# nv-tlabs/InfiniCube

Measured on AMD Instinct MI355X. Metric: denoise steps/sec, 93-frame 480p Wan2.1 buffer-conditioned DiT loop, higher is better.
Workload: dtype bf16

## Files before the change

infinicube_amd/csrc/attention.hip:

```cpp
#include "icv_common.h"


int icv_attn1_dispatch(const void* q, int64_t ldq, const void* k, int64_t ldk, const void* v, int64_t ldv, void* o,
                       int64_t ldo, int64_t Sq, int64_t Skv, int64_t heads, float scale, void* stream);
int icv_attn2_dispatch(const void* q, int64_t ldq, const void* k, int64_t ldk, const void* v, int64_t ldv,
                       void* o, int64_t ldo, float* acc, int64_t ldacc, float* ml, int state_in,
                       int state_out, int64_t Sq, int64_t Skv, int64_t heads, float scale, int var,
                       hipStream_t st);

int icv_attn3_dispatch(const void* q, int64_t ldq, const void* k, int64_t ldk, const void* v, int64_t ldv,
                       void* o, int64_t ldo, float* acc, int64_t ldacc, float* ml, int state_in,
                       int state_out, int64_t Sq, int64_t Skv, int64_t heads, float scale, int var,
                       hipStream_t st);

int icv_attn9_dispatch(const void* q, int64_t ldq, const void* k, int64_t ldk, const void* v, int64_t ldv,
                       void* o, int64_t ldo, float* acc, int64_t ldacc, float* ml, int state_in,
                       int state_out, int64_t Sq, int64_t Skv, int64_t heads, float scale, int var,
                       hipStream_t st);
int icv_attn7p_single(const void* q, int64_t ldq, const void* k, int64_t ldk, const void* v, int64_t ldv, void* o, int64_t ldo, float* acc,
                      int64_t ldacc, float* ml, int state_in, int state_out, int64_t Sq, int64_t Skv, int64_t heads, float scale, hipStream_t st);
int icv_attn7q_single(const void* q, int64_t ldq, const void* k, int64_t ldk, const void* v, int64_t ldv, void* o, int64_t ldo, float* acc,
                      int64_t ldacc, float* ml, int state_in, int state_out, int64_t Sq, int64_t Skv, int64_t heads, float scale, int variant,
                      hipStream_t st);
int icv_attn7_dispatch(const void* q, int64_t ldq, const void* k, int64_t ldk, const void* v, int64_t ldv,
// ... 70 lines not shown
                                 int64_t Skv, int64_t heads, float scale, void* stream) {
  ICV_REQUIRE(q && k && v && o, "icv_attention_fwd: null pointer");
  ICV_REQUIRE(Sq > 0 && Skv > 0 && heads > 0, "icv_attention_fwd: empty problem (Sq=%lld Skv=%lld heads=%lld)", (long long)Sq, (long long)Skv, (long long)heads);
  ICV_REQUIRE(ldq % 8 == 0 && ldk % 8 == 0 && ldv % 8 == 0 && ldo % 4 == 0, "icv_attention_fwd: leading dims must keep 16-byte row alignment");
  if (icv_get_option_int("attn_kernel", ATTN_KERNEL_DEFAULT) != 1)
    return attn_route(q, ldq, k, ldk, v, ldv, o, ldo, nullptr, 0, nullptr, 0, 0, Sq, Skv, heads, scale, (hipStream_t)stream);
#ifdef ICV_EXPERIMENTS
  return icv_attn1_dispatch(q, ldq, k, ldk, v, ldv, o, ldo, Sq, Skv, heads, scale, stream);
#else
  icv_set_error("attn_kernel 1 is an experiment: rebuild libicvideo with ICV_EXPERIMENTS=1");
  return 1;
#endif
}

extern "C" int icv_attention_fwd_add(const void* q, int64_t ldq, const void* k, int64_t ldk,
                                     const void* v, int64_t ldv, void* o, int64_t ldo, int64_t Sq,
                                     int64_t Skv, int64_t heads, float scale, void* stream) {
  ICV_REQUIRE(q && k && v && o, "icv_attention_fwd_add: null pointer");
  ICV_REQUIRE(Sq > 0 && Skv > 0 && heads > 0, "icv_attention_fwd_add: empty problem (Sq=%lld Skv=%lld heads=%lld)", (long long)Sq, (long long)Skv, (long long)heads);
  ICV_REQUIRE(ldq % 8 == 0 && ldk % 8 == 0 && ldv % 8 == 0 && ldo % 4 == 0, "icv_attention_fwd_add: leading dims must keep 16-byte row alignment");
  return attn_route(q, ldq, k, ldk, v, ldv, o, ldo, nullptr, 0, nullptr, 0, 2, Sq, Skv, heads, scale, (hipStream_t)stream);
}

namespace {
unsigned long long* g_trace = nullptr;
int g_trace_cap = 0;
}
unsigned long long* icv_attention_trace_buffer(int* capacity) {
  *capacity = g_trace_cap;
  return g_trace;
}
extern "C" int icv_attention_trace(void* buf, int64_t capacity) {
  ICV_REQUIRE(capacity >= 0 && capacity < (1LL << 31), "icv_attention_trace: bad capacity");
  g_trace = (unsigned long long*)buf;
  g_trace_cap = buf ? (int)capacity : 0;
  return 0;
}
```

infinicube_amd/csrc/attn7.hip:

```cpp
#include "attn_common.h"

namespace att7 {

using attc::D;
using attc::NEG_BIG;
using attc::Params;
using attc::lds_read_tr16;
constexpr int KVB = 64;
constexpr int TILE_BYTES = KVB * D * 2;
constexpr int STAGE_BYTES = 2 * TILE_BYTES;

__device__ __forceinline__ void dma16(const void* gsrc, unsigned lds_dst) {
  unsigned keep;
  asm volatile(
      "s_mov_b32 %0, m0\n\t"
      "s_mov_b32 m0, %2\n\t"
      "s_nop 0\n\t"
      "global_load_lds_dwordx4 %1, off\n\t"
      "s_mov_b32 m0, %0"
      : "=&s"(keep)
      : "v"(gsrc), "s"(lds_dst)
      : "memory");
}

__device__ __forceinline__ void dma16s(const void* base, unsigned off, unsigned lds_dst) {
  unsigned keep;
  asm volatile(
      "s_mov_b32 %0, m0\n\t"
      "s_mov_b32 m0, %3\n\t"
      "s_nop 0\n\t"
      "global_load_lds_dwordx4 %1, %2\n\t"
      "s_mov_b32 m0, %0"
      : "=&s"(keep)
      : "v"(off), "s"(base), "s"(lds_dst)
      : "memory");
}

#ifndef ATTN7_SHORT_DEFAULT
#define ATTN7_SHORT_DEFAULT 1024
#endif

template <int VAR, int NW, int NST>
__global__ __launch_bounds__(NW * 64) __attribute__((amdgpu_waves_per_eu(2))) void attn7_kernel(Params p) {
  constexpr bool STAGGER = VAR & 1, KPREFETCH = VAR & 2, SETPRIO = VAR & 4, DEEP = VAR & 8, UNIT = VAR & 16;
  constexpr bool DSMAJOR = !(VAR & 32);
  constexpr bool PAIR = (VAR & 128) != 0;
  static_assert(!(PAIR && (STAGGER || DEEP)), "the paired schedule has its own DMA distance");
  static_assert(!(STAGGER && DEEP), "the staggered group already runs its DMA three tiles ahead");
  static_assert(NST == 4 || !(PAIR || STAGGER || DEEP), "the two-stage ring has one schedule");
  static_assert(NW == 8 || !STAGGER, "the stagger pairs waves 0-3 with 4-7");
  constexpr int NI = 16 / NW;
  constexpr int QB = NW * 32;
  const float p_lim = __builtin_amdgcn_exp2f(p.thr);
  extern __shared__ __attribute__((aligned(16))) char smem[];
  const int tid = threadIdx.x;
  const int lane = tid & 63;
  const int wave = __builtin_amdgcn_readfirstlane(tid >> 6);
  const int hi = lane >> 5;
  const int l31 = lane & 31;

  int head, qb;
  attc::work_item(p, head, qb);
  const int64_t q0 = (int64_t)qb * QB + wave * 32;
  const unsigned long long t_start = p.trace ? __builtin_amdgcn_s_memrealtime() : 0ull;

  const bf16_t* qh = p.q + (int64_t)head * D;
  const bf16_t* kh = p.k + (int64_t)head * D;
  const bf16_t* vh = p.v + (int64_t)head * D;

  int64_t qr_c = q0 + l31;
  qr_c = qr_c < p.Sq ? qr_c : p.Sq - 1;

  f32x16 ot[4];
  float m_run, l_run;
  attc::load_state(p, qr_c, head, hi, ot, m_run, l_run);
  float m_base = m_run < -1.0e29f ? 0.f : m_run;
  f32x16 cinit;
  const f32x16 zero16 = {0.f, 0.f, 0.f, 0.f, 0.f, 0.f, 0.f, 0.f, 0.f, 0.f, 0.f, 0.f, 0.f, 0.f, 0.f, 0.f};
#pragma unroll
  for (int r = 0; r < 16; ++r) cinit[r] = UNIT ? -m_base : 0.f;

  bf16x8 qf[8];
#define A7_LOAD_Q()                                                                                   \
  {                                                                                                   \
    const bf16_t* qp = qh + qr_c * p.ldq + hi * 8;                                                    \
    _Pragma("unroll") for (int ds = 0; ds < 8; ++ds) qf[ds] = *reinterpret_cast<const bf16x8*>(qp + ds * 16); \
  }
  if (NST != 2) {
    A7_LOAD_Q();
    __builtin_amdgcn_s_waitcnt(0x0F70);
  }

  const int pc = lane & 15;
  const int nt = (int)((p.Skv + KVB - 1) / KVB);
  const unsigned lds_base = (unsigned)(uintptr_t)((__attribute__((address_space(3))) char*)smem);
  int dkey[NI], kcol[NI], vcol[NI];
  unsigned ko[NI], vo[NI];
#pragma unroll
  for (int j = 0; j < NI; ++j) {
    dkey[j] = (wave * NI + j) * 4 + (lane >> 4);
    kcol[j] = (pc ^ (dkey[j] & 15)) * 8;
    vcol[j] = (pc ^ ((dkey[j] & 3) << 2)) * 8;
    ko[j] = (unsigned)(((int64_t)dkey[j] * p.ldk + kcol[j]) * 2);
    vo[j] = (unsigned)(((int64_t)dkey[j] * p.ldv + vcol[j]) * 2);
  }
#define A7_DMA_TILE(T_)                                                                              \
  {                                                                                                  \
    const int tt_ = (T_) < nt ? (T_) : nt - 1;                                                       \
    const unsigned l0_ = lds_base + (unsigned)(((T_) & (NST - 1)) * STAGE_BYTES + (wave * NI) * 1024); \
    if ((int64_t)(tt_ + 1) * KVB <= p.Skv) {                                                         \
      const bf16_t* kt_ = kh + (int64_t)tt_ * KVB * p.ldk;                                           \
      const bf16_t* vt_ = vh + (int64_t)tt_ * KVB * p.ldv;                                           \
      _Pragma("unroll") for (int j_ = 0; j_ < NI; ++j_) dma16s(kt_, ko[j_], l0_ + j_ * 1024);        \
      _Pragma("unroll") for (int j_ = 0; j_ < NI; ++j_) dma16s(vt_, vo[j_], l0_ + TILE_BYTES + j_ * 1024); \
    } else {                                                                                         \
      _Pragma("unroll") for (int j_ = 0; j_ < NI; ++j_) {                                            \
        int64_t r_ = (int64_t)tt_ * KVB + dkey[j_];                                                  \
        r_ = r_ < p.Skv ? r_ : p.Skv - 1;                                                            \
        dma16(kh + r_ * p.ldk + kcol[j_], l0_ + j_ * 1024);                                          \
        dma16(vh + r_ * p.ldv + vcol[j_], l0_ + TILE_BYTES + j_ * 1024);                             \
      }                                                                                              \
    }                                                                                                \
  }
#define A7_VMCNT4()                                              \
  do {                                                           \
// ... 17 lines not shown
    A7_LOAD_Q();
    asm volatile("s_waitcnt vmcnt(0)" ::: "memory");
  } else if (PAIR) asm volatile("s_waitcnt vmcnt(0)" ::: "memory");
  else A7_VMCNT4();
  A7_BARRIER();
  if (grp == 1) {
    A7_DMA_TILE(2);
    A7_VMCNT4();
    A7_BARRIER();
  }

  const int k_row_off = l31 * 256;
  const int k_sw = l31 & 15;
  const int g = lane >> 4, t16 = lane & 15;
  const int v_key_lo = 4 * hi + (t16 >> 2);
  const int v_byte_lo = (g & 1) * 32 + (t16 & 3) * 8;
  const int v_sw = (t16 >> 2) << 6;
  const int ahead = 2 + grp + (DEEP ? 1 : 0);

  auto tile = [&](const int t) __attribute__((always_inline)) {
    const char* ks = smem + (t & (NST - 1)) * STAGE_BYTES;
    const char* vs = ks + TILE_BYTES;
    const int64_t key0 = (int64_t)t * KVB;

    f32x16 st[2];
    const bool no_ref = UNIT && m_run < -1.0e29f;
    if (KPREFETCH) {
      bf16x8 kf[2][8];
#pragma unroll
      for (int kb = 0; kb < 2; ++kb)
#pragma unroll
        for (int ds = 0; ds < 8; ++ds) {
          const int c = ds * 2 + hi;
          kf[kb][ds] = *reinterpret_cast<const bf16x8*>(ks + kb * 8192 + k_row_off + ((c ^ k_sw) << 4));
        }
      __builtin_amdgcn_sched_barrier(0);
      if (SETPRIO) __builtin_amdgcn_s_setprio(1);
#pragma unroll
      for (int ds = 0; ds < 8; ++ds)
#pragma unroll
        for (int kb = 0; kb < 2; ++kb)
          st[kb] = __builtin_amdgcn_mfma_f32_32x32x16_bf16(kf[kb][ds], qf[ds], ds == 0 ? (UNIT ? cinit : zero16) : st[kb], 0, 0, 0);
      if (SETPRIO) __builtin_amdgcn_s_setprio(0);
    } else if (DSMAJOR) {
#pragma unroll
      for (int ds = 0; ds < 8; ++ds)
// ... 103 lines not shown
    }
  } else if (PAIR) {
    for (int t = 0; t < nt; t += 2) {
      if (!(p.ablate & 1)) {
        A7_DMA_TILE(t + 2);
        A7_DMA_TILE(t + 3);
      }
      tile(t);
      if (t + 1 < nt) tile(t + 1);
      asm volatile("s_waitcnt vmcnt(0)" ::: "memory");
      if (!(p.ablate & 2)) A7_BARRIER();
    }
  } else {
    for (int t = 0; t < nt; ++t) {
      if (!(p.ablate & 1)) A7_DMA_TILE(t + ahead);
      tile(t);
      A7_VMCNT4();
      if (!(p.ablate & 2)) A7_BARRIER();
    }
  }
  asm volatile("s_waitcnt vmcnt(0)" ::: "memory");
  if (grp == 0 && STAGGER) A7_BARRIER();

  attc::store_result(p, q0 + l31, head, hi, ot, m_run, l_run);
  if (p.trace && tid == 0 && (int)blockIdx.x < p.trace_cap) {
    unsigned hwid, xcc;
    asm volatile("s_getreg_b32 %0, hwreg(HW_REG_HW_ID)" : "=s"(hwid));
    asm volatile("s_getreg_b32 %0, hwreg(HW_REG_XCC_ID)" : "=s"(xcc));
    unsigned long long* t = p.trace + (size_t)blockIdx.x * 4;
    t[0] = t_start; t[1] = __builtin_amdgcn_s_memrealtime(); t[2] = hwid; t[3] = xcc;
  }
}

template <int VAR, int NW = 8, int NST = 4>
int launch(const Params& p, hipStream_t st) {
  constexpr int LDS_BYTES = NST * STAGE_BYTES;
  static icv_dev_flags attr_set = {};
  if (int rc = icv_ensure_dynamic_lds((const void*)attn7_kernel<VAR, NW, NST>, LDS_BYTES, &attr_set, "attn7")) return rc;
  const int64_t nwg = (int64_t)p.heads * p.nqb;
  hipLaunchKernelGGL((attn7_kernel<VAR, NW, NST>), dim3((unsigned)nwg), dim3(NW * 64), LDS_BYTES, st, p);
  return icv_check_launch("icv_attention(7)");
}

}

int icv_attn7_dispatch(const void* q, int64_t ldq, const void* k, int64_t ldk, const void* v, int64_t ldv,
                       void* o, int64_t ldo, float* acc, int64_t ldacc, float* ml, int state_in,
                       int state_out, int64_t Sq, int64_t Skv, int64_t heads, float scale, int var,
                       hipStream_t st) {
  att7::Params p;
  int short_max = icv_get_option_int("attn7_short", -1);
  if (short_max < 0) short_max = ATTN7_SHORT_DEFAULT;
  const bool short_kv = Skv <= short_max;
  attc::fill_params(p, q, ldq, k, ldk, v, ldv, o, ldo, acc, ldacc, ml, state_in, state_out, Sq, Skv, heads, scale, short_kv ? 128 : 256);
  if (p.sc == 1.0f && icv_get_option_int("attn_unit_scale", 1)) var |= 16;
  p.ablate = icv_get_option_int("attn7_ablate", 0);
  p.trace = icv_attention_trace_buffer(&p.trace_cap);
  if (short_kv) return (var & 16) ? att7::launch<16, 4, 2>(p, st) : att7::launch<0, 4, 2>(p, st);
  switch (var) {
    case 0: return att7::launch<0>(p, st);
    case 1: return att7::launch<1>(p, st);
    case 4: return att7::launch<4>(p, st);
    case 5: return att7::launch<5>(p, st);
    case 6: return att7::launch<6>(p, st);
    case 7: return att7::launch<7>(p, st);
    case 8: return att7::launch<8>(p, st);
    case 24: return att7::launch<24>(p, st);
    case 32: return att7::launch<32>(p, st);
    case 48: return att7::launch<48>(p, st);
    case 128: return att7::launch<128>(p, st);
    case 144: return att7::launch<144>(p, st);
    case 132: return att7::launch<132>(p, st);
    case 148: return att7::launch<148>(p, st);
    case 16: return att7::launch<16>(p, st);
    case 17: return att7::launch<17>(p, st);
    case 20: return att7::launch<20>(p, st);
    case 21: return att7::launch<21>(p, st);
    case 22: return att7::launch<22>(p, st);
    case 23: return att7::launch<23>(p, st);
  }
  icv_set_error("icv_attention_fwd: unknown attn7 variant %d", var);
  return 1;
}
```

infinicube_amd/csrc/attn7p.hip:

```cpp
#include "attn_common.h"

namespace att7p {

using attc::D;
using attc::NEG_BIG;
using attc::lds_read_tr16;
constexpr int KVB = 64;
constexpr int TILE_BYTES = KVB * D * 2;
constexpr int STAGE_BYTES = 2 * TILE_BYTES;
constexpr int NST = 4, NW = 8, NI = 16 / NW, QB = NW * 32;
constexpr int LDS_BYTES = NST * STAGE_BYTES + 64;
constexpr int MAX_PIECES = ICV_ATTN_MAX_PIECES;

struct Piece {
  const bf16_t* k;
  const bf16_t* v;
  int rows;
  int flag;
  unsigned value;
  int pad;
};

struct Params {
  attc::Params a;
// ... 18 lines not shown
      : "v"(gsrc), "s"(lds_dst)
      : "memory");
}

__device__ __forceinline__ void dma16s(const void* base, unsigned off, unsigned lds_dst) {
  unsigned keep;
  asm volatile(
      "s_mov_b32 %0, m0\n\t"
      "s_mov_b32 m0, %3\n\t"
      "s_nop 0\n\t"
      "global_load_lds_dwordx4 %1, %2\n\t"
      "s_mov_b32 m0, %0"
      : "=&s"(keep)
      : "v"(off), "s"(base), "s"(lds_dst)
      : "memory");
}

__device__ __forceinline__ unsigned load_flag_async(const unsigned* f) {
  unsigned v;
  asm volatile("global_load_dword %0, %1, off sc0 sc1" : "=v"(v) : "v"(f) : "memory");
  return v;
}

template <bool UNIT, bool FW = false>
__global__ __launch_bounds__(NW * 64) __attribute__((amdgpu_waves_per_eu(2))) void attn7p_kernel(Params pp) {
  const attc::Params& p = pp.a;
  const float p_lim = __builtin_amdgcn_exp2f(p.thr);
  extern __shared__ __attribute__((aligned(16))) char smem[];
  volatile unsigned* verdict = reinterpret_cast<volatile unsigned*>(smem + NST * STAGE_BYTES);
  const int tid = threadIdx.x;
  const int lane = tid & 63;
  const int wave = __builtin_amdgcn_readfirstlane(tid >> 6);
  const int hi = lane >> 5;
  const int l31 = lane & 31;

  int head, qb;
  attc::work_item(p, head, qb);
  int64_t q0 = (int64_t)qb * QB + wave * 32;
  int64_t q_end = 0;
  int fw_np = 1, fw_a0 = 0, fw_b0 = 0, fw_a1 = 0, fw_b1 = 0;
  if constexpr (FW) {
    const int T = pp.fw_frames, F = pp.fw_frame_rows, W = pp.fw_window, sink = pp.fw_sink;
    const int bpf = (F + QB - 1) / QB;
    const int f = qb / bpf;
    q0 = (int64_t)f * F + (qb - f * bpf) * QB + wave * 32;
    q_end = (int64_t)(f + 1) * F;
    const int lo = f - W > 0 ? f - W : 0;
    const int hi = f + W + 1 < T ? f + W + 1 : T;
    if (sink == 0) {
      fw_a0 = lo; fw_b0 = hi;
    } else if (lo <= sink) {
      fw_a0 = 0; fw_b0 = hi > sink ? hi : sink;
    } else {
      fw_np = 2;
      fw_a0 = 0; fw_b0 = sink;
      fw_a1 = lo; fw_b1 = hi;
    }
  }
  const unsigned long long t_start = p.trace ? __builtin_amdgcn_s_memrealtime() : 0ull;
  const bf16_t* qh = p.q + (int64_t)head * D;
  int64_t qr_c = q0 + l31;
  if constexpr (FW) qr_c = qr_c < q_end ? qr_c : q_end - 1;
  else qr_c = qr_c < p.Sq ? qr_c : p.Sq - 1;

  f32x16 ot[4];
  float m_run, l_run;
  attc::load_state(p, qr_c, head, hi, ot, m_run, l_run);
  float m_base = m_run < -1.0e29f ? 0.f : m_run;
  f32x16 cinit;
  const f32x16 zero16 = {0.f, 0.f, 0.f, 0.f, 0.f, 0.f, 0.f, 0.f, 0.f, 0.f, 0.f, 0.f, 0.f, 0.f, 0.f, 0.f};
#pragma unroll
  for (int r = 0; r < 16; ++r) cinit[r] = UNIT ? -m_base : 0.f;

  bf16x8 qf[8];
  {
    const bf16_t* qp = qh + qr_c * p.ldq + hi * 8;
#pragma unroll
    for (int ds = 0; ds < 8; ++ds) qf[ds] = *reinterpret_cast<const bf16x8*>(qp + ds * 16);
  }
  __builtin_amdgcn_s_waitcnt(0x0F70);

  const int pc = lane & 15;
  const unsigned lds_base = (unsigned)(uintptr_t)((__attribute__((address_space(3))) char*)smem);
  int dkey[NI], kcol[NI], vcol[NI];
  unsigned ko[NI], vo[NI];
#pragma unroll
  for (int j = 0; j < NI; ++j) {
    dkey[j] = (wave * NI + j) * 4 + (lane >> 4);
    kcol[j] = (pc ^ (dkey[j] & 15)) * 8;
    vcol[j] = (pc ^ ((dkey[j] & 3) << 2)) * 8;
    ko[j] = (unsigned)(((int64_t)dkey[j] * p.ldk + kcol[j]) * 2);
    vo[j] = (unsigned)(((int64_t)dkey[j] * p.ldv + vcol[j]) * 2);
  }

  const bf16_t* kh_d = nullptr;
  const bf16_t* vh_d = nullptr;
  int skv_d = 0, nt_d = 0;
#define P_ROWS(J_) (FW ? ((J_) ? fw_b1 - fw_a1 : fw_b0 - fw_a0) * pp.fw_frame_rows : __builtin_amdgcn_readfirstlane(pp.piece[FW ? 0 : (J_)].rows))
#define P_SET_DMA_PIECE(J_)                                              \
  {                                                                      \
    if constexpr (FW) {                                                  \
      const int64_t r0_ = (int64_t)((J_) ? fw_a1 : fw_a0) * pp.fw_frame_rows; \
      kh_d = p.k + r0_ * p.ldk + (int64_t)head * D;                      \
      vh_d = p.v + r0_ * p.ldv + (int64_t)head * D;                      \
      skv_d = P_ROWS(J_);                                                \
    } else {                                                             \
      const Piece& pc_ = pp.piece[(J_)];                                 \
      kh_d = pc_.k + (int64_t)head * D;                                  \
      vh_d = pc_.v + (int64_t)head * D;                                  \
      skv_d = __builtin_amdgcn_readfirstlane(pc_.rows);                  \
    }                                                                    \
    nt_d = (skv_d + KVB - 1) / KVB;                                      \
  }
// ... 33 lines not shown
          __builtin_amdgcn_s_sleep(16);                                                                           \
              \
          if (pp.err && __hip_atomic_load(pp.err, __ATOMIC_RELAXED, __HIP_MEMORY_SCOPE_AGENT) != 0u) break;       \
          if (pp.timeout_ticks && __builtin_amdgcn_s_memrealtime() - t0_ > pp.timeout_ticks) {                    \
            if (pp.err) atomicCAS(pp.err, 0u, 0x80000000u | (unsigned)(J_));                                      \
            break;                                                                                                \
          }                                                                                                       \
        }                                                                                                         \
      }                                                                                                           \
      P_BARRIER();                                                                                                \
    }                                                                                                             \
  }

  const int k_row_off = l31 * 256;
  const int k_sw = l31 & 15;
  const int g = lane >> 4, t16 = lane & 15;
  const int v_key_lo = 4 * hi + (t16 >> 2);
  const int v_byte_lo = (g & 1) * 32 + (t16 & 3) * 8;
  const int v_sw = (t16 >> 2) << 6;

  auto tile = [&](const int stg, const int key0, const int skv) __attribute__((always_inline)) {
    const char* ks = smem + (stg & (NST - 1)) * STAGE_BYTES;
    const char* vs = ks + TILE_BYTES;
    f32x16 st[2];
    const bool no_ref = UNIT && m_run < -1.0e29f;
#pragma unroll
    for (int ds = 0; ds < 8; ++ds)
#pragma unroll
      for (int kb = 0; kb < 2; ++kb) {
        const int c = ds * 2 + hi;
        const bf16x8 kf = *reinterpret_cast<const bf16x8*>(ks + kb * 8192 + k_row_off + ((c ^ k_sw) << 4));
        st[kb] = __builtin_amdgcn_mfma_f32_32x32x16_bf16(kf, qf[ds], ds == 0 ? (UNIT ? cinit : zero16) : st[kb], 0, 0, 0);
      }
    if (key0 + KVB > skv) {
#pragma unroll
      for (int kb = 0; kb < 2; ++kb)
#pragma unroll
        for (int r = 0; r < 16; ++r) {
          const int key = key0 + kb * 32 + (r & 3) + 8 * (r >> 2) + 4 * hi;
          if (key >= skv) st[kb][r] = NEG_BIG;
        }
    }
    float mb = -m_run * p.sc;
    float psum = 0.f;
    __builtin_amdgcn_s_setprio(1);
#pragma unroll
// ... 44 lines not shown
      }
      psum += ps;
#pragma unroll
      for (int hf = 0; hf < 2; ++hf) {
        const int kk = kb * 2 + hf;
#pragma unroll
        for (int d0 = 0; d0 < 4; ++d0) {
          const int key_l = kk * 16 + v_key_lo;
          const int byte = (d0 * 64 + v_byte_lo) ^ v_sw;
          const bf16x4 va = lds_read_tr16(vs + key_l * 256 + byte);
          const bf16x4 vb = lds_read_tr16(vs + (key_l + 8) * 256 + byte);
          bf16x8 vf;
          vf[0] = va[0]; vf[1] = va[1]; vf[2] = va[2]; vf[3] = va[3];
          vf[4] = vb[0]; vf[5] = vb[1]; vf[6] = vb[2]; vf[7] = vb[3];
          ot[d0] = __builtin_amdgcn_mfma_f32_32x32x16_bf16(vf, pf[hf], ot[d0], 0, 0, 0);
        }
      }
    }
    __builtin_amdgcn_s_setprio(0);
    l_run += psum;
  };

  const int np = FW ? fw_np : __builtin_amdgcn_readfirstlane(pp.n_pieces);
  unsigned gt = 0;
  unsigned iv = 0;
  P_WAIT_PIECE(0);
  P_SET_DMA_PIECE(0);
  P_DMA_TILE(0, gt);
  P_DMA_TILE(1, gt + 1);
  asm volatile("s_waitcnt vmcnt(0)" ::: "memory");
  P_BARRIER();
  for (int pj = 0; pj < np; ++pj) {
    const int skv = P_ROWS(pj);
    const int nt = (skv + KVB - 1) / KVB;
    const unsigned g_next = gt + (unsigned)((nt + 1) & ~1);
    const bool has_next = pj + 1 < np;
    const int nflag = has_next && !FW ? __builtin_amdgcn_readfirstlane(pp.piece[has_next ? pj + 1 : pj].flag) : -1;
    const unsigned nvalue = has_next && !FW ? pp.piece[has_next ? pj + 1 : pj].value : 0u;
    bool next_ready = has_next && nflag < 0;
    bool next_issued = false;
    if (!FW && pp.ptrace && tid == 0) pp.ptrace[(size_t)blockIdx.x * np + pj] = __builtin_amdgcn_s_memrealtime();
    for (int t = 0; t < nt; t += 2) {
      const bool last_iv = t + 2 >= nt;
      if (!last_iv) {
        P_DMA_TILE(t + 2, gt + t + 2);
        P_DMA_TILE(t + 3, gt + t + 3);
      } else if (has_next && next_ready) {
        P_SET_DMA_PIECE(pj + 1);
        P_DMA_TILE(0, g_next);
        P_DMA_TILE(1, g_next + 1);
        next_issued = true;
      }
      const bool poll = has_next && !next_ready;
      unsigned fv = 0;
      if (poll && wave == 0) fv = load_flag_async(pp.flags + nflag);
      tile((int)(gt + t), t * KVB, skv);
      if (t + 1 < nt) tile((int)(gt + t + 1), (t + 1) * KVB, skv);
      asm volatile("s_waitcnt vmcnt(0)" ::: "memory");
      if (poll && tid == 0) verdict[iv & 1] = (int)(fv - nvalue) >= 0 ? 1u : 0u;
      P_BARRIER();
      if (poll) next_ready = __builtin_amdgcn_readfirstlane(verdict[iv & 1]) != 0;
      ++iv;
    }
    if (!has_next) break;
    if (!next_issued) {
      if (!next_ready) P_WAIT_PIECE(pj + 1);
      P_SET_DMA_PIECE(pj + 1);
      P_DMA_TILE(0, g_next);
      P_DMA_TILE(1, g_next + 1);
      asm volatile("s_waitcnt vmcnt(0)" ::: "memory");
      P_BARRIER();
    }
    gt = g_next;
  }
  asm volatile("s_waitcnt vmcnt(0)" ::: "memory");

  attc::store_result(p, !FW || q0 + l31 < q_end ? q0 + l31 : p.Sq, head, hi, ot, m_run, l_run);
  if (p.trace && tid == 0 && (int)blockIdx.x < p.trace_cap) {
    unsigned hwid, xcc;
    asm volatile("s_getreg_b32 %0, hwreg(HW_REG_HW_ID)" : "=s"(hwid));
    asm volatile("s_getreg_b32 %0, hwreg(HW_REG_XCC_ID)" : "=s"(xcc));
    unsigned long long* t = p.trace + (size_t)blockIdx.x * 4;
    t[0] = t_start; t[1] = __builtin_amdgcn_s_memrealtime(); t[2] = hwid; t[3] = xcc;
  }
#undef P_ROWS
#undef P_SET_DMA_PIECE
#undef P_DMA_TILE
#undef P_BARRIER
#undef P_WAIT_PIECE
}

template <bool UNIT, bool FW = false>
int launch(const Params& pp, hipStream_t st) {
  static icv_dev_flags attr_set = {};
  if (int rc = icv_ensure_dynamic_lds((const void*)attn7p_kernel<UNIT, FW>, LDS_BYTES, &attr_set, "attn7p")) return rc;
  const int64_t nwg = (int64_t)pp.a.heads * pp.a.nqb;
  hipLaunchKernelGGL((attn7p_kernel<UNIT, FW>), dim3((unsigned)nwg), dim3(NW * 64), LDS_BYTES, st, pp);
  return icv_check_launch(FW ? "icv_attention_fwd_framewin" : "icv_attention_fwd_pieces");
}

}

extern "C" int icv_attention_fwd_pieces(const void* q, int64_t ldq, const icv_kv_piece* pieces, int64_t n_pieces, int64_t ldk, int64_t ldv,
                                        void* o, int64_t ldo, int64_t Sq, int64_t heads, float scale, const uint32_t* flags, uint32_t* err,
                                        int64_t timeout_us, void* trace, void* stream) {
  ICV_REQUIRE(q && pieces && o, "icv_attention_fwd_pieces: null pointer");
  ICV_REQUIRE(Sq > 0 && heads > 0 && n_pieces > 0, "icv_attention_fwd_pieces: empty problem (Sq=%lld heads=%lld pieces=%lld)", (long long)Sq,
              (long long)heads, (long long)n_pieces);
  ICV_REQUIRE(ldq % 8 == 0 && ldk % 8 == 0 && ldv % 8 == 0 && ldo % 4 == 0, "icv_attention_fwd_pieces: leading dims must keep 16-byte row alignment");
  att7p::Params pp;
  int64_t total = 0;
  int n = 0;
  for (int64_t i = 0; i < n_pieces; ++i) {
    const icv_kv_piece& s = pieces[i];
    ICV_REQUIRE(s.rows >= 0 && s.rows < (1LL << 31) / 64, "icv_attention_fwd_pieces: piece %lld has %lld rows", (long long)i, (long long)s.rows);
    if (s.rows == 0) continue;
    ICV_REQUIRE(n < att7p::MAX_PIECES, "icv_attention_fwd_pieces: more than %d non-empty pieces", att7p::MAX_PIECES);
    ICV_REQUIRE(s.k && s.v, "icv_attention_fwd_pieces: piece %lld has a null pointer", (long long)i);
    ICV_REQUIRE(s.flag < 0 || flags, "icv_attention_fwd_pieces: piece %lld waits for flag %d but no flag array was given", (long long)i, s.flag);
    ICV_REQUIRE(64 * ldk * 2 < (1LL << 32) && 64 * ldv * 2 < (1LL << 32), "icv_attention_fwd_pieces: row stride too large");
    att7p::Piece& d = pp.piece[n++];
// ... 72 lines not shown
```

infinicube_amd/csrc/attn_common.h:

```cpp
#pragma once
#include "icv_common.h"

unsigned long long* icv_attention_trace_buffer(int* capacity);

namespace attc {

constexpr int D = 128;
constexpr float NEG_BIG = -1.0e30f;

struct Params {
  const bf16_t* q; int64_t ldq;
  const bf16_t* k; int64_t ldk;
  const bf16_t* v; int64_t ldv;
  bf16_t* o; int64_t ldo;
  float* acc; int64_t ldacc;
  float* ml;
  int64_t Sq, Skv;
  int heads, nqb;
  int state_in, state_out;
  float sc;
  float thr;
  int ablate;
  unsigned long long* trace;
  int trace_cap;
};

// ... 67 lines not shown
      for (int rr = 0; rr < 4; ++rr)
        *reinterpret_cast<float4*>(ap + d0 * 32 + rr * 8) =
            make_float4(ot[d0][rr * 4 + 0], ot[d0][rr * 4 + 1], ot[d0][rr * 4 + 2], ot[d0][rr * 4 + 3]);
    if (hi == 0) *reinterpret_cast<float2*>(p.ml + (qr * p.heads + head) * 2) = make_float2(m_run, l_tot);
  } else {
    const float inv = 1.0f / l_tot;
    bf16_t* op = p.o + qr * p.ldo + (int64_t)head * D + 4 * hi;
#pragma unroll
    for (int d0 = 0; d0 < 4; ++d0)
#pragma unroll
      for (int rr = 0; rr < 4; ++rr) {
        float a = ot[d0][rr * 4 + 0] * inv, b = ot[d0][rr * 4 + 1] * inv;
        float c = ot[d0][rr * 4 + 2] * inv, d = ot[d0][rr * 4 + 3] * inv;
        if (p.state_out == 2) {
          const uint2 prev = *reinterpret_cast<const uint2*>(op + d0 * 32 + rr * 8);
          a += __uint_as_float(prev.x << 16); b += __uint_as_float(prev.x & 0xFFFF0000u);
          c += __uint_as_float(prev.y << 16); d += __uint_as_float(prev.y & 0xFFFF0000u);
        }
        *reinterpret_cast<uint2*>(op + d0 * 32 + rr * 8) = make_uint2(pack_bf16x2(a, b), pack_bf16x2(c, d));
      }
  }
}

}
```

Before: 0.2973.

## Switch attention kernels to 16x16x32 MFMA tiles by default

Adds a 16x16x32 bf16 MFMA path for the attn7 and attn7p flash-attention kernels, processing each 32-row query block as two 16-row sub-tiles with new LDS swizzles, transposed V reads and per-subtile online softmax state. The shape is chosen with a runtime option and defaults to 16 for both short and long KV. The intent is to use the higher-throughput 16x16 MFMA shape and get better instruction scheduling on MI355X. In exchange it doubles the softmax bookkeeping, adds extra cross-lane shuffles, and may change register pressure.

Result: faster. 0.3012 (median of 6 runs) (+1.3%).

```diff
diff --git a/infinicube_amd/csrc/attention.hip b/infinicube_amd/csrc/attention.hip
--- a/infinicube_amd/csrc/attention.hip
+++ b/infinicube_amd/csrc/attention.hip
@@ -116,6 +116,16 @@
   return attn_route(q, ldq, k, ldk, v, ldv, o, ldo, nullptr, 0, nullptr, 0, 2, Sq, Skv, heads, scale, (hipStream_t)stream);
 }
 
+constexpr int ATTN_MFMA_DEFAULT = 16;
+constexpr int ATTN_MFMA_SHORT_DEFAULT = 16;
+int icv_attn_mfma(bool short_kv) {
+  const int v = icv_get_option_int("attn_mfma", -1);
+  if (v < 0) return short_kv ? ATTN_MFMA_SHORT_DEFAULT : ATTN_MFMA_DEFAULT;
+  if (v == 16 || v == 32) return v;
+  icv_set_error("attn_mfma = %d: the MFMA shape is 16 (16x16x32) or 32 (32x32x16); negative = the default", v);
+  return -1;
+}
+
 namespace {
 unsigned long long* g_trace = nullptr;
 int g_trace_cap = 0;
diff --git a/infinicube_amd/csrc/attn7.hip b/infinicube_amd/csrc/attn7.hip
--- a/infinicube_amd/csrc/attn7.hip
+++ b/infinicube_amd/csrc/attn7.hip
@@ -40,8 +40,9 @@
 #define ATTN7_SHORT_DEFAULT 1024
 #endif
 
-template <int VAR, int NW, int NST>
+template <int VAR, int NW, int NST, int MF>
 __global__ __launch_bounds__(NW * 64) __attribute__((amdgpu_waves_per_eu(2))) void attn7_kernel(Params p) {
+  static_assert(MF == 16 || MF == 32, "MF: 16 (16x16x32 MFMAs) or 32 (32x32x16)");
   constexpr bool STAGGER = VAR & 1, KPREFETCH = VAR & 2, SETPRIO = VAR & 4, DEEP = VAR & 8, UNIT = VAR & 16;
   constexpr bool DSMAJOR = !(VAR & 32);
   constexpr bool PAIR = (VAR & 128) != 0;
@@ -72,8 +73,19 @@
   qr_c = qr_c < p.Sq ? qr_c : p.Sq - 1;
 
   f32x16 ot[4];
-  float m_run, l_run;
-  attc::load_state(p, qr_c, head, hi, ot, m_run, l_run);
+  float m_run = NEG_BIG, l_run = 0.f;
+  attc::Tile16 s16;
+  int64_t qr16[2] = {0, 0};
+  if constexpr (MF == 16) {
+#pragma unroll
+    for (int qb = 0; qb < 2; ++qb) {
+      const int64_t r = q0 + qb * 16 + (lane & 15);
+      qr16[qb] = r < p.Sq ? r : p.Sq - 1;
+    }
+    attc::tile16_init<UNIT>(p, qr16, head, lane >> 4, s16);
+  } else {
+    attc::load_state(p, qr_c, head, hi, ot, m_run, l_run);
+  }
   float m_base = m_run < -1.0e29f ? 0.f : m_run;
   f32x16 cinit;
   const f32x16 zero16 = {0.f, 0.f, 0.f, 0.f, 0.f, 0.f, 0.f, 0.f, 0.f, 0.f, 0.f, 0.f, 0.f, 0.f, 0.f, 0.f};
@@ -82,7 +94,8 @@
 
   bf16x8 qf[8];
 #define A7_LOAD_Q()                                                                                   \
-  {                                                                                                   \
+  if constexpr (MF == 16) attc::tile16_load_q(p, qr16, head, lane >> 4, s16);                          \
+  else {                                                                                              \
     const bf16_t* qp = qh + qr_c * p.ldq + hi * 8;                                                    \
     _Pragma("unroll") for (int ds = 0; ds < 8; ++ds) qf[ds] = *reinterpret_cast<const bf16x8*>(qp + ds * 16); \
   }
@@ -100,7 +113,7 @@
   for (int j = 0; j < NI; ++j) {
     dkey[j] = (wave * NI + j) * 4 + (lane >> 4);
     kcol[j] = (pc ^ (dkey[j] & 15)) * 8;
-    vcol[j] = (pc ^ ((dkey[j] & 3) << 2)) * 8;
+    vcol[j] = MF == 16 ? attc::tile16_vcol(pc, dkey[j]) : (pc ^ ((dkey[j] & 3) << 2)) * 8;
     ko[j] = (unsigned)(((int64_t)dkey[j] * p.ldk + kcol[j]) * 2);
     vo[j] = (unsigned)(((int64_t)dkey[j] * p.ldv + vcol[j]) * 2);
   }
@@ -164,6 +177,10 @@
     const char* ks = smem + (t & (NST - 1)) * STAGE_BYTES;
     const char* vs = ks + TILE_BYTES;
     const int64_t key0 = (int64_t)t * KVB;
+    if constexpr (MF == 16) {
+      attc::tile16<UNIT, KPREFETCH, DSMAJOR, SETPRIO>(p, p_lim, ks, vs, key0, p.Skv, lane, s16);
+      return;
+    }
 
     f32x16 st[2];
     const bool no_ref = UNIT && m_run < -1.0e29f;
@@ -313,7 +330,14 @@
   asm volatile("s_waitcnt vmcnt(0)" ::: "memory");
   if (grp == 0 && STAGGER) A7_BARRIER();
 
-  attc::store_result(p, q0 + l31, head, hi, ot, m_run, l_run);
+  if constexpr (MF == 16) {
+    int t16 = lane & 15;
+    asm volatile("" : "+v"(t16));
+    const int64_t qr[2] = {q0 + t16, q0 + 16 + t16};
+    attc::store_result(p, qr, head, lane >> 4, s16.ot, s16.m_run, s16.l_run);
+  } else {
+    attc::store_result(p, q0 + l31, head, hi, ot, m_run, l_run);
+  }
   if (p.trace && tid == 0 && (int)blockIdx.x < p.trace_cap) {
     unsigned hwid, xcc;
     asm volatile("s_getreg_b32 %0, hwreg(HW_REG_HW_ID)" : "=s"(hwid));
@@ -323,14 +347,19 @@
   }
 }
 
-template <int VAR, int NW = 8, int NST = 4>
-int launch(const Params& p, hipStream_t st) {
+template <int VAR, int NW, int NST, int MF>
+int launch_mf(const Params& p, hipStream_t st) {
   constexpr int LDS_BYTES = NST * STAGE_BYTES;
   static icv_dev_flags attr_set = {};
-  if (int rc = icv_ensure_dynamic_lds((const void*)attn7_kernel<VAR, NW, NST>, LDS_BYTES, &attr_set, "attn7")) return rc;
+  if (int rc = icv_ensure_dynamic_lds((const void*)attn7_kernel<VAR, NW, NST, MF>, LDS_BYTES, &attr_set, "attn7")) return rc;
   const int64_t nwg = (int64_t)p.heads * p.nqb;
-  hipLaunchKernelGGL((attn7_kernel<VAR, NW, NST>), dim3((unsigned)nwg), dim3(NW * 64), LDS_BYTES, st, p);
+  hipLaunchKernelGGL((attn7_kernel<VAR, NW, NST, MF>), dim3((unsigned)nwg), dim3(NW * 64), LDS_BYTES, st, p);
   return icv_check_launch("icv_attention(7)");
+}
+
+template <int VAR, int NW = 8, int NST = 4>
+int launch(const Params& p, hipStream_t st, int mf) {
+  return mf == 16 ? launch_mf<VAR, NW, NST, 16>(p, st) : launch_mf<VAR, NW, NST, 32>(p, st);
 }
 
 }
@@ -347,28 +376,30 @@
   if (p.sc == 1.0f && icv_get_option_int("attn_unit_scale", 1)) var |= 16;
   p.ablate = icv_get_option_int("attn7_ablate", 0);
   p.trace = icv_attention_trace_buffer(&p.trace_cap);
-  if (short_kv) return (var & 16) ? att7::launch<16, 4, 2>(p, st) : att7::launch<0, 4, 2>(p, st);
+  const int mf = icv_attn_mfma(short_kv);
+  if (mf < 0) return 1;
+  if (short_kv) return (var & 16) ? att7::launch<16, 4, 2>(p, st, mf) : att7::launch<0, 4, 2>(p, st, mf);
   switch (var) {
-    case 0: return att7::launch<0>(p, st);
-    case 1: return att7::launch<1>(p, st);
-    case 4: return att7::launch<4>(p, st);
-    case 5: return att7::launch<5>(p, st);
-    case 6: return att7::launch<6>(p, st);
-    case 7: return att7::launch<7>(p, st);
-    case 8: return att7::launch<8>(p, st);
-    case 24: return att7::launch<24>(p, st);
-    case 32: return att7::launch<32>(p, st);
-    case 48: return att7::launch<48>(p, st);
-    case 128: return att7::launch<128>(p, st);
-    case 144: return att7::launch<144>(p, st);
-    case 132: return att7::launch<132>(p, st);
-    case 148: return att7::launch<148>(p, st);
-    case 16: return att7::launch<16>(p, st);
-    case 17: return att7::launch<17>(p, st);
-    case 20: return att7::launch<20>(p, st);
-    case 21: return att7::launch<21>(p, st);
-    case 22: return att7::launch<22>(p, st);
-    case 23: return att7::launch<23>(p, st);
+    case 0: return att7::launch<0>(p, st, mf);
+    case 1: return att7::launch<1>(p, st, mf);
+    case 4: return att7::launch<4>(p, st, mf);
+    case 5: return att7::launch<5>(p, st, mf);
+    case 6: return att7::launch<6>(p, st, mf);
+    case 7: return att7::launch<7>(p, st, mf);
+    case 8: return att7::launch<8>(p, st, mf);
+    case 24: return att7::launch<24>(p, st, mf);
+    case 32: return att7::launch<32>(p, st, mf);
+    case 48: return att7::launch<48>(p, st, mf);
+    case 128: return att7::launch<128>(p, st, mf);
+    case 144: return att7::launch<144>(p, st, mf);
+    case 132: return att7::launch<132>(p, st, mf);
+    case 148: return att7::launch<148>(p, st, mf);
+    case 16: return att7::launch<16>(p, st, mf);
+    case 17: return att7::launch<17>(p, st, mf);
+    case 20: return att7::launch<20>(p, st, mf);
+    case 21: return att7::launch<21>(p, st, mf);
+    case 22: return att7::launch<22>(p, st, mf);
+    case 23: return att7::launch<23>(p, st, mf);
   }
   icv_set_error("icv_attention_fwd: unknown attn7 variant %d", var);
   return 1;
diff --git a/infinicube_amd/csrc/attn7p.hip b/infinicube_amd/csrc/attn7p.hip
--- a/infinicube_amd/csrc/attn7p.hip
+++ b/infinicube_amd/csrc/attn7p.hip
@@ -64,8 +64,9 @@
   return v;
 }
 
-template <bool UNIT, bool FW = false>
+template <bool UNIT, bool FW, int MF>
 __global__ __launch_bounds__(NW * 64) __attribute__((amdgpu_waves_per_eu(2))) void attn7p_kernel(Params pp) {
+  static_assert(MF == 16 || MF == 32, "MF: 16 (16x16x32 MFMAs) or 32 (32x32x16)");
   const attc::Params& p = pp.a;
   const float p_lim = __builtin_amdgcn_exp2f(p.thr);
   extern __shared__ __attribute__((aligned(16))) char smem[];
@@ -106,8 +107,20 @@
   else qr_c = qr_c < p.Sq ? qr_c : p.Sq - 1;
 
   f32x16 ot[4];
-  float m_run, l_run;
-  attc::load_state(p, qr_c, head, hi, ot, m_run, l_run);
+  float m_run = NEG_BIG, l_run = 0.f;
+  attc::Tile16 s16;
+  int64_t qr16[2] = {0, 0};
+  if constexpr (MF == 16) {
+    const int64_t q_lim = FW ? q_end : p.Sq;
+#pragma unroll
+    for (int qb = 0; qb < 2; ++qb) {
+      const int64_t r = q0 + qb * 16 + (lane & 15);
+      qr16[qb] = r < q_lim ? r : q_lim - 1;
+    }
+    attc::tile16_init<UNIT>(p, qr16, head, lane >> 4, s16);
+  } else {
+    attc::load_state(p, qr_c, head, hi, ot, m_run, l_run);
+  }
   float m_base = m_run < -1.0e29f ? 0.f : m_run;
   f32x16 cinit;
   const f32x16 zero16 = {0.f, 0.f, 0.f, 0.f, 0.f, 0.f, 0.f, 0.f, 0.f, 0.f, 0.f, 0.f, 0.f, 0.f, 0.f, 0.f};
@@ -115,7 +128,8 @@
   for (int r = 0; r < 16; ++r) cinit[r] = UNIT ? -m_base : 0.f;
 
   bf16x8 qf[8];
-  {
+  if constexpr (MF == 16) attc::tile16_load_q(p, qr16, head, lane >> 4, s16);
+  else {
     const bf16_t* qp = qh + qr_c * p.ldq + hi * 8;
 #pragma unroll
     for (int ds = 0; ds < 8; ++ds) qf[ds] = *reinterpret_cast<const bf16x8*>(qp + ds * 16);
@@ -130,7 +144,7 @@
   for (int j = 0; j < NI; ++j) {
     dkey[j] = (wave * NI + j) * 4 + (lane >> 4);
     kcol[j] = (pc ^ (dkey[j] & 15)) * 8;
-    vcol[j] = (pc ^ ((dkey[j] & 3) << 2)) * 8;
+    vcol[j] = MF == 16 ? attc::tile16_vcol(pc, dkey[j]) : (pc ^ ((dkey[j] & 3) << 2)) * 8;
     ko[j] = (unsigned)(((int64_t)dkey[j] * p.ldk + kcol[j]) * 2);
     vo[j] = (unsigned)(((int64_t)dkey[j] * p.ldv + vcol[j]) * 2);
   }
@@ -210,6 +224,10 @@
   auto tile = [&](const int stg, const int key0, const int skv) __attribute__((always_inline)) {
     const char* ks = smem + (stg & (NST - 1)) * STAGE_BYTES;
     const char* vs = ks + TILE_BYTES;
+    if constexpr (MF == 16) {
+      attc::tile16<UNIT, false, true, true>(p, p_lim, ks, vs, key0, skv, lane, s16);
+      return;
+    }
     f32x16 st[2];
     const bool no_ref = UNIT && m_run < -1.0e29f;
 #pragma unroll
@@ -300,6 +318,7 @@
   };
 
   const int np = FW ? fw_np : __builtin_amdgcn_readfirstlane(pp.n_pieces);
+  if constexpr (MF == 16) __builtin_assume(np >= 1);
   unsigned gt = 0;
   unsigned iv = 0;
   P_WAIT_PIECE(0);
@@ -311,6 +330,7 @@
   for (int pj = 0; pj < np; ++pj) {
     const int skv = P_ROWS(pj);
     const int nt = (skv + KVB - 1) / KVB;
+    if constexpr (MF == 16) __builtin_assume(nt >= 1);
     const unsigned g_next = gt + (unsigned)((nt + 1) & ~1);
     const bool has_next = pj + 1 < np;
     const int nflag = has_next && !FW ? __builtin_amdgcn_readfirstlane(pp.piece[has_next ? pj + 1 : pj].flag) : -1;
@@ -353,7 +373,19 @@
   }
   asm volatile("s_waitcnt vmcnt(0)" ::: "memory");
 
-  attc::store_result(p, !FW || q0 + l31 < q_end ? q0 + l31 : p.Sq, head, hi, ot, m_run, l_run);
+  if constexpr (MF == 16) {
+    int64_t qr[2];
+    int t16 = lane & 15;
+    asm volatile("" : "+v"(t16));
+#pragma unroll
+    for (int qb = 0; qb < 2; ++qb) {
+      const int64_t r = q0 + qb * 16 + t16;
+      qr[qb] = !FW || r < q_end ? r : p.Sq;
+    }
+    attc::store_result(p, qr, head, lane >> 4, s16.ot, s16.m_run, s16.l_run);
+  } else {
+    attc::store_result(p, !FW || q0 + l31 < q_end ? q0 + l31 : p.Sq, head, hi, ot, m_run, l_run);
+  }
   if (p.trace && tid == 0 && (int)blockIdx.x < p.trace_cap) {
     unsigned hwid, xcc;
     asm volatile("s_getreg_b32 %0, hwreg(HW_REG_HW_ID)" : "=s"(hwid));
@@ -368,13 +400,20 @@
 #undef P_WAIT_PIECE
 }
 
+template <bool UNIT, bool FW, int MF>
+int launch_mf(const Params& pp, hipStream_t st) {
+  static icv_dev_flags attr_set = {};
+  if (int rc = icv_ensure_dynamic_lds((const void*)attn7p_kernel<UNIT, FW, MF>, LDS_BYTES, &attr_set, "attn7p")) return rc;
+  const int64_t nwg = (int64_t)pp.a.heads * pp.a.nqb;
+  hipLaunchKernelGGL((attn7p_kernel<UNIT, FW, MF>), dim3((unsigned)nwg), dim3(NW * 64), LDS_BYTES, st, pp);
+  return icv_check_launch(FW ? "icv_attention_fwd_framewin" : "icv_attention_fwd_pieces");
+}
+
 template <bool UNIT, bool FW = false>
 int launch(const Params& pp, hipStream_t st) {
-  static icv_dev_flags attr_set = {};
-  if (int rc = icv_ensure_dynamic_lds((const void*)attn7p_kernel<UNIT, FW>, LDS_BYTES, &attr_set, "attn7p")) return rc;
-  const int64_t nwg = (int64_t)pp.a.heads * pp.a.nqb;
-  hipLaunchKernelGGL((attn7p_kernel<UNIT, FW>), dim3((unsigned)nwg), dim3(NW * 64), LDS_BYTES, st, pp);
-  return icv_check_launch(FW ? "icv_attention_fwd_framewin" : "icv_attention_fwd_pieces");
+  const int mf = icv_attn_mfma(false);
+  if (mf < 0) return 1;
+  return mf == 16 ? launch_mf<UNIT, FW, 16>(pp, st) : launch_mf<UNIT, FW, 32>(pp, st);
 }
 
 }
diff --git a/infinicube_amd/csrc/attn_common.h b/infinicube_amd/csrc/attn_common.h
--- a/infinicube_amd/csrc/attn_common.h
+++ b/infinicube_amd/csrc/attn_common.h
@@ -2,6 +2,7 @@
 #include "icv_common.h"
 
 unsigned long long* icv_attention_trace_buffer(int* capacity);
+int icv_attn_mfma(bool short_kv);
 
 namespace attc {
 
@@ -115,4 +116,245 @@
   }
 }
 
-}
+struct Tile16 {
+  f32x4 ot[8][2];
+  float m_run[2], l_run[2], m_base[2];
+  f32x4 cinit[2];
+  bf16x8 qf[2][4];
+};
+
+__device__ __forceinline__ void load_state(const Params& p, const int64_t (&qr_c)[2], int head, int g, f32x4 (&ot)[8][2],
+                                           float (&m_run)[2], float (&l_run)[2]) {
+#pragma unroll
+  for (int qb = 0; qb < 2; ++qb) {
+    if (p.state_in) {
+      const float* ap = p.acc + qr_c[qb] * p.ldacc + (int64_t)head * D + 4 * g;
+#pragma unroll
+      for (int db = 0; db < 8; ++db) {
+        const float4 a = *reinterpret_cast<const float4*>(ap + db * 16);
+        ot[db][qb][0] = a.x; ot[db][qb][1] = a.y; ot[db][qb][2] = a.z; ot[db][qb][3] = a.w;
+      }
+      const float2 mlv = *reinterpret_cast<const float2*>(p.ml + (qr_c[qb] * p.heads + head) * 2);
+      m_run[qb] = mlv.x;
+      l_run[qb] = g == 0 ? mlv.y : 0.f;
+    } else {
+#pragma unroll
+      for (int db = 0; db < 8; ++db)
+#pragma unroll
+        for (int r = 0; r < 4; ++r) ot[db][qb][r] = 0.f;
+      m_run[qb] = NEG_BIG;
+      l_run[qb] = 0.f;
+    }
+  }
+}
+
+__device__ __forceinline__ void store_result(const Params& p, const int64_t (&qr)[2], int head, int g, const f32x4 (&ot)[8][2],
+                                             const float (&m_run)[2], const float (&l_run)[2]) {
+  float l_tot[2];
+#pragma unroll
+  for (int qb = 0; qb < 2; ++qb) {
+    const float l2 = l_run[qb] + __shfl_xor(l_run[qb], 16, 64);
+    l_tot[qb] = l2 + __shfl_xor(l2, 32, 64);
+  }
+#pragma unroll
+  for (int qb = 0; qb < 2; ++qb) {
+    if (qr[qb] >= p.Sq) continue;
+    if (p.state_out == 1) {
+      float* ap = p.acc + qr[qb] * p.ldacc + (int64_t)head * D + 4 * g;
+#pragma unroll
+      for (int db = 0; db < 8; ++db)
+        *reinterpret_cast<float4*>(ap + db * 16) = make_float4(ot[db][qb][0], ot[db][qb][1], ot[db][qb][2], ot[db][qb][3]);
+      if (g == 0) *reinterpret_cast<float2*>(p.ml + (qr[qb] * p.heads + head) * 2) = make_float2(m_run[qb], l_tot[qb]);
+    } else {
+      const float inv = 1.0f / l_tot[qb];
+      bf16_t* op = p.o + qr[qb] * p.ldo + (int64_t)head * D + 4 * g;
+#pragma unroll
+      for (int db = 0; db < 8; ++db) {
+        float a = ot[db][qb][0] * inv, b = ot[db][qb][1] * inv;
+        float c = ot[db][qb][2] * inv, d = ot[db][qb][3] * inv;
+        if (p.state_out == 2) {
+          const uint2 prev = *reinterpret_cast<const uint2*>(op + db * 16);
+          a += __uint_as_float(prev.x << 16); b += __uint_as_float(prev.x & 0xFFFF0000u);
+          c += __uint_as_float(prev.y << 16); d += __uint_as_float(prev.y & 0xFFFF0000u);
+        }
+        *reinterpret_cast<uint2*>(op + db * 16) = make_uint2(pack_bf16x2(a, b), pack_bf16x2(c, d));
+      }
+    }
+  }
+}
+
+__device__ __forceinline__ void tile16_load_q(const Params& p, const int64_t (&qr_c)[2], int head, int g, Tile16& s) {
+  const bf16_t* qh = p.q + (int64_t)head * D + g * 8;
+#pragma unroll
+  for (int qb = 0; qb < 2; ++qb)
+#pragma unroll
+    for (int ks = 0; ks < 4; ++ks) s.qf[qb][ks] = *reinterpret_cast<const bf16x8*>(qh + qr_c[qb] * p.ldq + ks * 32);
+}
+
+template <bool UNIT>
+__device__ __forceinline__ void tile16_init(const Params& p, const int64_t (&qr_c)[2], int head, int g, Tile16& s) {
+  load_state(p, qr_c, head, g, s.ot, s.m_run, s.l_run);
+#pragma unroll
+  for (int qb = 0; qb < 2; ++qb) {
+    s.m_base[qb] = s.m_run[qb] < -1.0e29f ? 0.f : s.m_run[qb];
+#pragma unroll
+    for (int r = 0; r < 4; ++r) s.cinit[qb][r] = UNIT ? -s.m_base[qb] : 0.f;
+  }
+}
+
+__device__ __forceinline__ int tile16_vcol(int pc, int key) { return (pc ^ ((key & 7) << 1)) * 8; }
+
+template <bool UNIT, bool KPREFETCH, bool DSMAJOR, bool SETPRIO>
+__device__ __forceinline__ void tile16(const Params& p, const float p_lim, const char* ks, const char* vs, const int64_t key0,
+                                       const int64_t skv, const int lane, Tile16& s) {
+  const int g = lane >> 4, t = lane & 15;
+  const f32x4 zero4 = {0.f, 0.f, 0.f, 0.f};
+  const int k_row_off = t * 256;
+  const int v_row_off = (4 * g + (t >> 2)) * 256;
+  const int v_sw = (4 * (g & 1) + (t >> 2)) << 5;
+  const int v_byte_lo = (t & 3) * 8;
+  f32x4 st[4][2];
+  const bool no_ref = UNIT && (s.m_run[0] < -1.0e29f || s.m_run[1] < -1.0e29f);
+#define T16_KADDR(KB_, KS_) (ks + (KB_) * 4096 + k_row_off + ((((KS_) * 4 + g) ^ t) << 4))
+#define T16_QK(KB_, KS_, KF_)                                                                                       \
+  _Pragma("unroll") for (int qb = 0; qb < 2; ++qb) st[KB_][qb] = __builtin_amdgcn_mfma_f32_16x16x32_bf16(           \
+      KF_, s.qf[qb][KS_], (KS_) == 0 ? (UNIT ? s.cinit[qb] : zero4) : st[KB_][qb], 0, 0, 0)
+  if (KPREFETCH) {
+    bf16x8 kf[4][4];
+#pragma unroll
+    for (int kb = 0; kb < 4; ++kb)
+#pragma unroll
+      for (int kq = 0; kq < 4; ++kq) kf[kb][kq] = *reinterpret_cast<const bf16x8*>(T16_KADDR(kb, kq));
+    __builtin_amdgcn_sched_barrier(0);
+    if (SETPRIO) __builtin_amdgcn_s_setprio(1);
+#pragma unroll
+    for (int kq = 0; kq < 4; ++kq)
+#pragma unroll
+      for (int kb = 0; kb < 4; ++kb) { T16_QK(kb, kq, kf[kb][kq]); }
+    if (SETPRIO) __builtin_amdgcn_s_setprio(0);
+  } else if (DSMAJOR) {
+    constexpr int KD = 3;
+    bf16x8 kf[16];
+#pragma unroll
+    for (int i = 0; i < KD; ++i) kf[i] = *reinterpret_cast<const bf16x8*>(T16_KADDR(i & 3, i >> 2));
+#pragma unroll
+    for (int i = 0; i < 16; ++i) {
+      if (i + KD < 16) kf[i + KD] = *reinterpret_cast<const bf16x8*>(T16_KADDR((i + KD) & 3, (i + KD) >> 2));
+      T16_QK(i & 3, i >> 2, kf[i]);
+    }
+    __builtin_amdgcn_sched_group_barrier(0x100, KD, 0);
+#pragma unroll
+    for (int i = 0; i < 16; ++i) {
+      if (i + KD < 16) __builtin_amdgcn_sched_group_barrier(0x100, 1, 0);
+      __builtin_amdgcn_sched_group_barrier(0x008, 2, 0);
+    }
+  } else {
+    if (SETPRIO) __builtin_amdgcn_s_setprio(1);
+#pragma unroll
+    for (int kb = 0; kb < 4; ++kb)
+#pragma unroll
+      for (int kq = 0; kq < 4; ++kq) {
+        const bf16x8 kf = *reinterpret_cast<const bf16x8*>(T16_KADDR(kb, kq));
+        T16_QK(kb, kq, kf);
+      }
+    if (SETPRIO) __builtin_amdgcn_s_setprio(0);
+  }
+#undef T16_KADDR
+#undef T16_QK
+  if (key0 + 64 > skv) {
+#pragma unroll
+    for (int kb = 0; kb < 4; ++kb)
+#pragma unroll
+      for (int r = 0; r < 4; ++r) {
+        const int64_t key = key0 + kb * 16 + 4 * g + r;
+        if (key >= skv) { st[kb][0][r] = NEG_BIG; st[kb][1][r] = NEG_BIG; }
+      }
+  }
+  float mb[2] = {-s.m_run[0] * p.sc, -s.m_run[1] * p.sc};
+  float psum[2] = {0.f, 0.f};
+  if (SETPRIO) __builtin_amdgcn_s_setprio(1);
+#pragma unroll
+  for (int kk = 0; kk < 2; ++kk) {
+    bf16x8 pf[2];
+    float ps[2];
+#define T16_EXP()                                                                                                   \
+  _Pragma("unroll") for (int qb = 0; qb < 2; ++qb) {                                                                \
+    ps[qb] = 0.f;                                                                                                   \
+    _Pragma("unroll") for (int j = 0; j < 8; ++j) {                                                                 \
+      const float sv = st[2 * kk + (j >> 2)][qb][j & 3];                                                            \
+      const float pv = UNIT ? __builtin_amdgcn_exp2f(sv) : __builtin_amdgcn_exp2f(fmaf(sv, p.sc, mb[qb]));          \
+      ps[qb] += pv;                                                                                                 \
+      pf[qb][j] = (__bf16)pv;                                                                                       \
+    }                                                                                                               \
+  }
+    T16_EXP();
+    if (__any(!(ps[0] <= p_lim) || !(ps[1] <= p_lim) || no_ref)) {
+#pragma unroll
+      for (int qb = 0; qb < 2; ++qb) {
+        float mloc = st[2 * kk][qb][0];
+#pragma unroll
+        for (int j = 1; j < 8; ++j) mloc = fmaxf(mloc, st[2 * kk + (j >> 2)][qb][j & 3]);
+        mloc = fmaxf(mloc, __shfl_xor(mloc, 16, 64));
+        mloc = fmaxf(mloc, __shfl_xor(mloc, 32, 64));
+        if (UNIT) mloc += s.m_base[qb];
+        const float m_new = fmaxf(s.m_run[qb], mloc);
+        const float alpha = __builtin_amdgcn_exp2f((s.m_run[qb] - m_new) * p.sc);
+        s.m_run[qb] = m_new;
+        s.l_run[qb] = (s.l_run[qb] + psum[qb]) * alpha;
+        psum[qb] = 0.f;
+#pragma unroll
+        for (int db = 0; db < 8; ++db)
+#pragma unroll
+          for (int r = 0; r < 4; ++r) s.ot[db][qb][r] *= alpha;
+        mb[qb] = -m_new * p.sc;
+        if (UNIT) {
+          const float dm = m_new - s.m_base[qb];
+          s.m_base[qb] = m_new;
+#pragma unroll
+          for (int kb = 0; kb < 4; ++kb)
+            if (kb >= 2 * kk) {
+#pragma unroll
+              for (int r = 0; r < 4; ++r) st[kb][qb][r] -= dm;
+            }
+#pragma unroll
+          for (int r = 0; r < 4; ++r) s.cinit[qb][r] = -m_new;
+        }
+      }
+      T16_EXP();
+    }
+#undef T16_EXP
+    psum[0] += ps[0];
+    psum[1] += ps[1];
+    constexpr int VD = 2;
+    bf16x4 va[8], vb[8];
+#define T16_VREAD(DB_)                                                                                  \
+  {                                                                                                     \
+    const char* va_p = vs + kk * 8192 + v_row_off + (((DB_) * 32 + v_byte_lo) ^ v_sw);                   \
+    va[DB_] = lds_read_tr16(va_p);                                                                      \
+    vb[DB_] = lds_read_tr16(va_p + 4096);  \
+  }
+#pragma unroll
+    for (int db = 0; db < VD; ++db) T16_VREAD(db);
+#pragma unroll
+    for (int db = 0; db < 8; ++db) {
+      if (db + VD < 8) T16_VREAD(db + VD);
+      bf16x8 vf;
+      vf[0] = va[db][0]; vf[1] = va[db][1]; vf[2] = va[db][2]; vf[3] = va[db][3];
+      vf[4] = vb[db][0]; vf[5] = vb[db][1]; vf[6] = vb[db][2]; vf[7] = vb[db][3];
+#pragma unroll
+      for (int qb = 0; qb < 2; ++qb) s.ot[db][qb] = __builtin_amdgcn_mfma_f32_16x16x32_bf16(vf, pf[qb], s.ot[db][qb], 0, 0, 0);
+    }
+#undef T16_VREAD
+    __builtin_amdgcn_sched_group_barrier(0x100, 2 * VD, 0);
+#pragma unroll
+    for (int db = 0; db < 8; ++db) {
+      if (db + VD < 8) __builtin_amdgcn_sched_group_barrier(0x100, 2, 0);
+      __builtin_amdgcn_sched_group_barrier(0x008, 2, 0);
+    }
+  }
+  if (SETPRIO) __builtin_amdgcn_s_setprio(0);
+  s.l_run[0] += psum[0];
+  s.l_run[1] += psum[1];
+}
+
+}
```
